# Complexity-ML/complexity-tokenizer

Measured on AMD Instinct MI355X. Metric: MB/s raw UTF-8 encoded (encode_batch), 50k ByteLevel BPE, 1/2/4/8 MI355X, higher is better.
Workload: dtype u8

## Files before the change

### complexity-tokenizer_amd/csrc/ctok_host.cpp

```cpp
#include <emmintrin.h>
#include <sched.h>
#include <hip/hip_runtime.h>

#include <algorithm>
#include <atomic>
#include <chrono>
#include <cstdio>
#include <cstring>
#include <exception>
#include <fstream>
#include <functional>
#include <map>
#include <memory>
#include <mutex>
#include <sstream>
#include <thread>
#include <string>
#include <string_view>
#include <unordered_map>
#include <unordered_set>
#include <vector>

#include "../../include/ctok.h"
#include "ctok_internal.h"
// ... 239 lines not shown
      (void)hipSetDevice(device);
      if (pipe) {
        for (int i = 0; i < 2; i++) {
          if (pipe->ev_h2d[i]) (void)hipEventDestroy(pipe->ev_h2d[i]);
          if (pipe->ev_enc[i]) (void)hipEventDestroy(pipe->ev_enc[i]);
          if (pipe->ev_d2h[i]) (void)hipEventDestroy(pipe->ev_d2h[i]);
        }
        for (auto& e : pipe->ev_t) if (e) (void)hipEventDestroy(e);
        if (pipe->up) (void)hipStreamDestroy(pipe->up);
        if (pipe->down) (void)hipStreamDestroy(pipe->down);
        pipe.reset();
      }
      for (auto& e : ev) if (e) (void)hipEventDestroy(e);
      for (auto& e : dev_ev) if (e) (void)hipEventDestroy(e);
      if (ev_sync) (void)hipEventDestroy(ev_sync);
      if (ev_join) (void)hipEventDestroy(ev_join);
      if (side) (void)hipStreamDestroy(side);
      if (ev_tot) (void)hipEventDestroy(ev_tot);
      if (host) (void)hipHostFree(host);
      if (stream) (void)hipStreamDestroy(stream);
    }
  }
};

}


struct ctok {
  std::unordered_map<std::string, uint32_t> vocab;
  std::unordered_map<uint32_t, std::string> id_to_token;
  std::vector<std::pair<std::string, uint32_t>> special;
  bool nfc = true;
  bool add_prefix_space = false;
  std::vector<uint64_t> merge_tab;
  uint32_t merge_mask = 0;
  std::vector<uint64_t> lds_image;
  std::vector<uint64_t> lds16_image, merge16;
  uint32_t merge16_mask = 0;
  std::vector<uint32_t> pair0;
  size_t hot_entries = 0;
  std::vector<uint32_t> piece_tab;
  uint32_t piece_mask = 0;
  std::vector<uint32_t> rank_newid;
  std::vector<uint32_t> eager_bits;
  std::vector<uint32_t> wmeta;
  bool window = false;
  int32_t byte2id[256];
  std::string at_bytes;
  std::vector<uint32_t> at_off{0}, at_id;
  std::vector<uint8_t> at_flags;
  bool proper = true;
  bool compact = false;
  bool narrow = false;
  bool ids16 = false;
  int decoder = 1;
  std::string decoder_name;
  std::vector<uint32_t> dec_ent;
  std::vector<uint8_t> dec_bytes;
  bool has_pp = false;
  std::vector<uint32_t> pp_items;
  int pp_kind = 0;
  std::string pp_single, pp_pair;
  bool pp_has_pair = false;
  uint64_t model_max_length = 512;
  std::mutex dev_mu;
  std::map<int, std::unique_ptr<DeviceState>> devs;
};

namespace {

bool get_bool_field(const ctj::Value& o, const char* k, bool dflt, const char* ctx) {
  const ctj::Value* v = o.get(k);
  if (!v) return dflt;
  if (v->kind != ctj::Value::Bool) throw_err(CTOK_E_PARSE, std::string("invalid type for `") + k + "` in " + ctx + ", expected a boolean");
  return v->b;
}

int parse_normalizer(const ctj::Value* v) {
  if (v && v->kind == ctj::Value::Object) {
    const ctj::Value* t = v->get("type");
    if (t) {
      std::string ty = t->kind == ctj::Value::String ? t->s : "";
      if (ty == "NFC") return 1;
      if (ty == "Sequence") {
        const ctj::Value* ns = v->get("normalizers");
        if (!ns || ns->kind != ctj::Value::Array) return 0;
        int any = 0;
        for (const auto& n : ns->arr) any |= parse_normalizer(&n);
        return any;
      }
      static const char* unsup[] = {"NFD", "NFKC", "NFKD", "Lowercase", "Strip", "StripAccents", "Replace",
                                    "Prepend", "BertNormalizer", "Precompiled"};
      for (const char* u : unsup)
        if (ty == u) throw_err(CTOK_E_UNSUPPORTED, "normalizer `" + ty + "` is outside the encode hot path (only NFC / none)");
      return 0;
    }
  }
  return 1;
}

bool is_white_space(uint32_t c) {
  return (c >= 9 && c <= 13) || c == 32 || c == 0x85 || c == 0xA0 || c == 0x1680 || (c >= 0x2000 && c <= 0x200A) ||
         c == 0x2028 || c == 0x2029 || c == 0x202F || c == 0x205F || c == 0x3000;
}

std::string encode_utf8(const std::vector<uint32_t>& cps, size_t a, size_t b) {
// ... 653 lines not shown
          const uint32_t v = t->compact ? z : r;
          t->eager_bits[v >> 5] |= 1u << (v & 31);
        }
      }
    }
  }


  {
    auto nchars = [&](uint32_t id, bool& ok) -> uint32_t {
      auto it = t->id_to_token.find(id);
      if (it == t->id_to_token.end()) { ok = false; return 0; }
      uint32_t c = 0;
      for (unsigned char ch : it->second) c += (ch & 0xC0) != 0x80;
      return c;
    };
    bool ok = !getenv("CTOK_NO_WINDOW");
    for (int b = 0; b < 256 && ok; b++)
      if (t->byte2id[b] >= 0 && nchars((uint32_t)t->byte2id[b], ok) != 1) ok = false;
    uint32_t max_id = 0;
    for (const auto& kv : t->vocab) max_id = std::max(max_id, kv.second);
    std::vector<uint32_t> ml, mr;
    if (ok) {
      ml.assign((size_t)max_id + 1, 0);
      mr.assign((size_t)max_id + 1, 0);
    }
    for (const auto& kv : ranks) {
      if (!ok) break;
      const uint32_t r = kv.second;
      if (r >= valid_new.size()) continue;
      const uint32_t a = (uint32_t)(kv.first >> 32), b = (uint32_t)kv.first;
      const uint32_t la = nchars(a, ok), lb = nchars(b, ok), lz = nchars(valid_new[r], ok);
      if (!ok || lz != la + lb || a > max_id || b > max_id) { ok = false; break; }
      ml[b] = std::max(ml[b], la);
      mr[a] = std::max(mr[a], lb);
    }
    t->window = ok;
    if (ok) {
      t->wmeta.resize((size_t)max_id + 1);
      for (size_t i = 0; i <= max_id; i++) t->wmeta[i] = std::min(ml[i], 0xFFFFu) | std::min(mr[i], 0xFFFFu) << 16;
    }
  }
  lap("window");

  t->pair0.assign(65536, kNoRank);
  for (uint32_t a = 0; a < 256; a++)
    for (uint32_t b = 0; b < 256; b++) {
      if (t->byte2id[a] < 0 || t->byte2id[b] < 0) continue;
      auto it = ranks.find(((uint64_t)(uint32_t)t->byte2id[a] << 32) | (uint32_t)t->byte2id[b]);
      if (it == ranks.end()) continue;
      const uint32_t r = it->second;
      t->pair0[a * 256 + b] = t->compact ? (r < valid_new.size() ? valid_new[r] : kPanicVal) : r;
    }

  lap("proper+pair0");
  {
    std::vector<int> inv0(0x144, -1);
    for (int b = 0; b < 256; b++) inv0[bm[b]] = b;
    auto tab_value = [&](uint32_t a, uint32_t b) -> uint64_t {
      const uint64_t key = ((uint64_t)a << kIdBits) | b;
      for (uint32_t h = mhash(a, b) & t->merge_mask;; h = (h + 1) & t->merge_mask) {
        const uint64_t e = t->merge_tab[h];
        if (e == kEmpty) return UINT64_MAX;
        if ((e & ((1ull << 42) - 1)) == key) return e >> 42;
      }
    };
    const uint64_t n_valid = valid_new.size();
    auto panics = [&](uint64_t v) { return t->compact ? v == kPanicVal : v >= n_valid; };
    std::vector<std::pair<const std::string*, uint32_t>> items;
    items.reserve(t->vocab.size());
    for (const auto& kv : t->vocab) items.push_back({&kv.first, kv.second});
    const unsigned nth = std::min(16u, usable_cpus_once());
    std::vector<std::vector<std::pair<std::string, uint32_t>>> part(nth);
    auto work = [&](unsigned w) {
      std::vector<uint32_t> cps, tk;
      for (size_t i = w; i < items.size(); i += nth) {
        const std::string& key = *items[i].first;
        if (!decode_utf8(key, cps) || cps.empty() || cps.size() > 8) continue;
        std::string raw;
        bool ok = true;
        for (uint32_t c : cps) {
          if (c >= inv0.size() || inv0[c] < 0) { ok = false; break; }
          raw += (char)inv0[c];
        }
        if (!ok) continue;
        tk.clear();
        for (unsigned char c : raw) {
          if (t->byte2id[c] < 0) { ok = false; break; }
          tk.push_back((uint32_t)t->byte2id[c]);
        }
        if (!ok) continue;
        for (;;) {
          size_t bi = 0;
          uint64_t best = UINT64_MAX;
          for (size_t j = 0; j + 1 < tk.size(); j++) {
            const uint64_t v = tab_value(tk[j], tk[j + 1]);
            if (v == UINT64_MAX) continue;
            if (panics(v)) { ok = false; break; }
            if (v < best) { best = v; bi = j; }
          }
          if (!ok || best == UINT64_MAX) break;
          tk[bi] = t->compact ? (uint32_t)best : valid_new[best];
          tk.erase(tk.begin() + bi + 1);
        }
        if (ok && tk.size() == 1 && tk[0] == items[i].second) part[w].push_back({raw, items[i].second});
      }
// ... 166 lines not shown
      return b;
    }();
    upload(ds->cls_bmp, bmp.data(), bmp.size(), s);
  }
  upload(ds->decomp_cp, ct_decomp_cp, CT_DECOMP_N, s);
  upload(ds->decomp_off, ct_decomp_off, CT_DECOMP_N + 1, s);
  upload(ds->decomp_data, ct_decomp_data, CT_DECOMP_DATA_N, s);
  upload(ds->comp_key, (const uint64_t*)ct_comp_key, CT_COMP_N, s);
  upload(ds->comp_val, ct_comp_val, CT_COMP_N, s);
  upload(ds->alnum, ct_bytemap_alnum, 256, s);
  upload(ds->at_bytes, (const uint8_t*)t->at_bytes.data(), t->at_bytes.size(), s);
  upload(ds->at_off, t->at_off.data(), t->at_off.size(), s);
  upload(ds->at_id, t->at_id.data(), t->at_id.size(), s);
  upload(ds->at_flags, t->at_flags.data(), t->at_flags.size(), s);
  HIPTRY(hipStreamSynchronize(s));
  Tables& tb = ds->t;
  tb.merge_tab = ds->merge_tab.p;
  tb.merge_mask = t->merge_mask;
  tb.lds_image = (const uint4*)ds->lds_image.p;
  tb.pair0 = ds->pair0.p;
  tb.lds16_image = (const uint4*)ds->lds16_image.p;
  tb.merge16 = ds->merge16.p;
  tb.merge16_mask = t->merge16_mask;
  tb.piece_tab = (const uint4*)ds->piece_tab.p;
  tb.piece_mask = t->piece_mask;
  tb.rank_newid = ds->rank_newid.p;
  tb.eager = ds->eager.p;
  tb.wmeta = ds->wmeta.p;
  tb.window = t->window ? 1 : 0;
  tb.n_ranks = (uint32_t)t->rank_newid.size();
  tb.byte2id = ds->byte2id.p;
  tb.cls_s1 = ds->cls_s1.p;
  tb.cls_s2 = ds->cls_s2.p;
  tb.nfc_s1 = ds->nfc_s1.p;
  tb.nfc_s2 = ds->nfc_s2.p;
  tb.cls_bmp = ds->cls_bmp.p;
  tb.cp_fast = cp_fast_ok() ? 1u : 0u;
  tb.decomp_cp = ds->decomp_cp.p;
  tb.decomp_off = ds->decomp_off.p;
  tb.decomp_data = ds->decomp_data.p;
  tb.n_decomp = CT_DECOMP_N;
  tb.comp_key = ds->comp_key.p;
  tb.comp_val = ds->comp_val.p;
  tb.n_comp = CT_COMP_N;
  tb.bytemap_alnum = ds->alnum.p;
  tb.at_bytes = ds->at_bytes.p;
  tb.at_off = ds->at_off.p;
  tb.at_id = ds->at_id.p;
  tb.at_flags = ds->at_flags.p;
  tb.n_at = (uint32_t)t->at_id.size();
  tb.proper = (t->proper && !getenv("CTOK_FORCE_IMPROPER")) ? 1 : 0;
  tb.compact = t->compact ? 1 : 0;
  tb.narrow = (t->narrow && !getenv("CTOK_FORCE_WIDE_SLOTS")) ? 1 : 0;
  tb.all_bytes = std::all_of(t->byte2id, t->byte2id + 256, [](int32_t v) { return v >= 0; }) ? 1 : 0;
  tb.dbg = getenv("CTOK_DBG_MODE") ? (uint32_t)atoi(getenv("CTOK_DBG_MODE")) : 0;
  DeviceState* r = ds.get();
  t->devs[device] = std::move(ds);
  return r;
}

bool debug_sync() {
  static int v = -1;
  if (v < 0) v = getenv("CTOK_DEBUG_SYNC") ? 1 : 0;
  return v == 1;
}

#define STEP(name, x)                                                                    \
  do {                                                                                   \
    HIPTRY(x);                                                                           \
    if (debug_sync()) {                                                                  \
      fprintf(stderr, "[ctok] %s launched\n", name);                                     \
      HIPTRY(hipStreamSynchronize(s));                                                   \
      fprintf(stderr, "[ctok] %s done\n", name);                                         \
    }                                                                                    \
  } while (0)

template <class Idle>
void spin_sync(DeviceState* ds, hipStream_t s, Idle idle) {
  HIPTRY(hipEventRecord(ds->ev_sync, s));
  for (;;) {
    hipError_t e = hipEventQuery(ds->ev_sync);
    if (e == hipSuccess) return;
    if (e != hipErrorNotReady) throw_err(CTOK_E_DEVICE, std::string("hipEventQuery: ") + hipGetErrorString(e));
    idle();
  }
}
void spin_sync(DeviceState* ds, hipStream_t s) {
  spin_sync(ds, s, [] {});
}

struct Laps {
  struct Lap {
    hipEvent_t a, b;
    double v;
    bool done;
  };
  Lap l[12];
  int n = 0;
  int add(hipEvent_t a, hipEvent_t b) {
    l[n] = {a, b, 0.0, false};
    return n++;
  }
  void read(Lap& p) {
    float v = 0;
    HIPTRY(hipEventElapsedTime(&v, p.a, p.b));
    p.v = v;
// ... 1615 lines not shown
```

### complexity-tokenizer_amd/csrc/ctok_internal.h

```cpp
#pragma once
#include <hip/hip_runtime.h>

#include <cstdint>

namespace ctok_dev {

constexpr uint64_t kEmpty = ~0ull;
constexpr uint32_t kIdBits = 21;
constexpr uint64_t kKeyMask = (1ull << 42) - 1;
constexpr uint32_t kNoRank = 0x3FFFFFu;
constexpr uint32_t kMaxId = (1u << kIdBits) - 2;
constexpr uint32_t kPanicVal = kNoRank - 1;

constexpr uint32_t kErrPanic = 1u;

constexpr int kTileWords = 62;
constexpr int kTile = kTileWords * 64;
constexpr int kTileSlots = 4096;
constexpr int kSegWaves = 4;
constexpr int kSegUnroll = 4;
constexpr int kShortMax = 32;
constexpr int kMedMax = 64;
constexpr uint32_t kCap0 = kTile, kCap1 = (kTile + 8) / 9, kCap2 = (kTile + 16) / 17, kCap3 = (kTile + 32) / 33;
constexpr uint32_t kCap0Lean = 1040;
// ... 73 lines not shown
  uint32_t h = mul24(lo, 0x9E3779u) + mul24((lo >> 24) | (hi << 8), 0x85EBCBu) + mul24((hi >> 16) | (len << 16), 0xC2B2AFu);
  h ^= h >> 15;
  h = mul24(h, 0x27D4EBu) ^ (h >> 9);
  return h ^ (h >> 16);
}

__host__ __device__ __forceinline__ int cp_range_class(uint32_t cp) {
  if (cp - 0x4E00u < 0x5200u) return 1;
  if (cp - 0xAC00u < 0x2BA4u) return 1;
  if (cp - 0x3041u < 0x56u) return 1;
  if (cp - 0x30A1u < 0x5Au) return 1;
  if (cp - 0x1F300u < 0x350u) return 3;
  return -1;
}

struct Tables {
  const uint64_t* merge_tab;
  uint32_t merge_mask;
  const uint4* lds_image;
  const uint32_t* pair0;
  const uint4* lds16_image;
  const uint64_t* merge16;
  uint32_t merge16_mask;
  const uint4* piece_tab;
  uint32_t piece_mask;
  const uint32_t* rank_newid;
  uint32_t n_ranks;
  const int32_t* byte2id;
  const uint8_t* cls_s1;
  const uint8_t* cls_s2;
  const uint8_t* nfc_s1;
  const uint16_t* nfc_s2;
  const uint8_t* cls_bmp;
  uint32_t cp_fast;
  const uint32_t* decomp_cp;
  const uint16_t* decomp_off;
  const uint32_t* decomp_data;
  uint32_t n_decomp;
  const uint64_t* comp_key;
  const uint32_t* comp_val;
  uint32_t n_comp;
  const uint8_t* bytemap_alnum;
  const uint8_t* at_bytes;
  const uint32_t* at_off;
  const uint32_t* at_id;
  const uint8_t* at_flags;
  uint32_t n_at;
  uint32_t proper;
  const uint32_t* eager;
  uint32_t window;
  const uint32_t* wmeta;
  uint32_t compact;
  uint32_t narrow;
  uint32_t dbg;
  uint32_t all_bytes;
};

struct Work {
  const uint8_t* text;
  uint32_t n_bytes;
  const uint64_t* doc_off;
  uint32_t n_docs;
  uint32_t* tfirst;
  uint32_t* pbits;
  uint32_t n_words;
  uint32_t n_tiles;
  uint32_t n_cus;
  uint32_t nfc_watch;
  uint32_t* nfc_bits;
  uint32_t mid_wide;
  uint32_t short_wgs;
  uint32_t keep_first;
  uint16_t* wpref;
  uint32_t* tile_np;
  uint32_t* tile_tok;
  uint32_t* tile_doc;
  uint32_t* tcls;
  uint32_t* list0;
  uint32_t k0;
  uint32_t* list1;
  uint32_t* list2;
  uint32_t* list3;
  void* prec;
  uint32_t rec16;
  uint32_t* mrec;
  uint32_t* pdoc;
  uint32_t* tcnt;
  uint32_t* long_cnt;
  uint32_t* long_ord;
  uint32_t* long_hist;
  uint32_t* scratch;
  uint32_t* lids;
  uint32_t* long_pos;
  uint32_t* lw_pos;
  uint32_t* rend;
  uint2* tregion;
  uint32_t long_cap, mid_cap;
  uint32_t unit;
  uint64_t* long_list;
  uint64_t* mid_list;
  uint32_t* counters;
  uint32_t* lw;
  uint32_t* scan_tmp;
  uint64_t scan_tmp_cap;
  uint64_t* stamps;
  uint32_t c3_max;
// ... 112 lines not shown
```

### complexity-tokenizer_amd/csrc/kernels.hip

```cpp
#include <hip/hip_ext.h>
#include <hip/hip_runtime.h>

#include <algorithm>
#include <mutex>
#include <type_traits>

#include "ctok_internal.h"
#include "seg_lane.h"

namespace ctok_dev {

#define HIPCHK(x) do { hipError_t e_ = (x); if (e_ != hipSuccess) return e_; } while (0)

template <typename F, typename... A>
static void launch_lx(const Lx& x, F k, dim3 grid, dim3 block, uint32_t lds, hipStream_t s, A... a) {
  if (x.start || x.stop)
    hipExtLaunchKernelGGL(k, grid, block, lds, s, x.start, x.stop, 0u, a...);
  else
    hipLaunchKernelGGL(k, grid, block, lds, s, a...);
}

constexpr uint32_t kNone = 0xFFFFFFFFu;
constexpr uint32_t kDead = 0xFFFFFFFFu;
constexpr uint32_t kSel = kNoRank - 1;


__device__ __forceinline__ void write_report(const Work& w) {
  const uint32_t lane = threadIdx.x & 63;
  uint32_t c3 = 0;
  if (w.c3_max) {
    const uint32_t c = w.counters[kNumCounters + lane];
    uint32_t inc = c;
#pragma unroll
    for (int o = 1; o < 64; o <<= 1) {
      const uint32_t v = (uint32_t)__shfl_up((int)inc, o, 64);
      if (lane >= (uint32_t)o) inc += v;
    }
    w.c3pre[lane] = inc - c;
    if (lane == 63) w.c3pre[64] = inc;
    c3 = __shfl((int)inc, 63, 64);
    if (__ballot(c > w.c3_max / kC3Shards)) c3 = ~0u;
  }
  if (lane < (uint32_t)kNumCounters) w.report[lane] = lane == (uint32_t)kCtrC3Count ? c3 : w.counters[lane];
  __builtin_amdgcn_fence(__ATOMIC_RELEASE, "");
  asm volatile("s_waitcnt vmcnt(0)" ::: "memory");
  if (lane == 0) __hip_atomic_store(&w.report[kNumCounters], w.seq, __ATOMIC_RELAXED, __HIP_MEMORY_SCOPE_SYSTEM);
  __builtin_amdgcn_fence(__ATOMIC_RELEASE, "");
}

__device__ __forceinline__ uint32_t wave_min_u32(uint32_t v) {
#pragma unroll
  for (int o = 32; o > 0; o >>= 1) v = min(v, (uint32_t)__shfl_xor((int)v, o, 64));
  return v;
}

__device__ __forceinline__ uint32_t wave_min_full_u32(uint32_t v) {
  v = min(v, (uint32_t)__builtin_amdgcn_update_dpp((int)v, (int)v, 0xB1, 0xF, 0xF, false));
  v = min(v, (uint32_t)__builtin_amdgcn_update_dpp((int)v, (int)v, 0x4E, 0xF, 0xF, false));
  v = min(v, (uint32_t)__builtin_amdgcn_update_dpp((int)v, (int)v, 0x141, 0xF, 0xF, false));
  v = min(v, (uint32_t)__builtin_amdgcn_update_dpp((int)v, (int)v, 0x140, 0xF, 0xF, false));
// ... 1052 lines not shown
template <> struct LdsClass<32> { static constexpr int cls = 2; static constexpr uint32_t cap = kCap2; };
template <> struct LdsClass<64> { static constexpr int cls = 3; static constexpr uint32_t cap = kCap3; };

template <int N>
__device__ __forceinline__ const uint32_t* class_list(const Work& w) {
  return N == 8 ? w.list0 : N == 16 ? w.list1 : N == 32 ? w.list2 : w.list3;
}
template <int N>
__device__ __forceinline__ uint32_t class_cap(const Work& w) {
  return N == 8 ? w.k0 : LdsClass<N>::cap;
}

template <int N, bool COMPACT, bool HOT, bool NARROW>
__device__ __forceinline__ bool merge_slots(const Tables& t, const PairLds& P, uint32_t* tk, uint32_t* rk,
                                            uint32_t& m, uint32_t stop, uint32_t* err) {
  for (;;) {
    if (m <= stop) return true;
    uint32_t key = ~0u;
#pragma unroll
    for (int k = 0; k < N - 1; k++) key = min(key, (rk[k] << 6) | (uint32_t)k);
    const uint32_t best = key >> 6, bi = key & 63u;
    if (best == kNoRank) return false;
    const uint32_t nid = COMPACT ? best : t.rank_newid[best];
    uint32_t L = 0, R = 0;
#pragma unroll
    for (int k = 0; k < N; k++) {
      L = ((uint32_t)k + 1 == bi) ? tk[k] : L;
      R = ((uint32_t)k == bi + 2) ? tk[k] : R;
    }
    const bool has_l = bi > 0, has_r = bi + 2 < m;
    Probe<NARROW, HOT> pl, pr;
    pl.start(t, P, L, nid, has_l);
    pr.start(t, P, nid, R, has_r);
#pragma unroll
    for (int k = 0; k < N; k++) {
      const uint32_t nxt_t = k + 1 < N ? tk[k + 1] : kDead;
      const uint32_t nxt_r = k + 1 < N ? rk[k + 1] : kNoRank;
      const bool gt = (uint32_t)k > bi;
      tk[k] = gt ? nxt_t : ((uint32_t)k == bi ? nid : tk[k]);
      rk[k] = gt ? nxt_r : rk[k];
    }
    m--;
    const uint32_t rl = has_l ? pl.finish(t, err) : kNoRank;
    const uint32_t rr = has_r ? pr.finish(t, err) : kNoRank;
#pragma unroll
    for (int k = 0; k < N - 1; k++)
      rk[k] = ((uint32_t)k + 1 == bi) ? rl : (((uint32_t)k == bi) ? rr : rk[k]);
  }
}

typedef __attribute__((address_space(3))) uint16_t lds_u16;

template <bool COMPACT, bool HOT, uint32_t NT, typename OutOf>
__device__ __forceinline__ uint32_t merge_lds8(const Tables& t, const PairLds& P, const uint32_t* tk, const uint32_t* rk,
                                               uint32_t m, lds_u32* s_key, lds_u16* s_tok, uint32_t* err,
                                               OutOf&& out_of) {
  const uint32_t tid = threadIdx.x;
#pragma unroll
  for (int k = 0; k < 8; k++) {
    s_key[k * NT + tid] = (uint32_t)k + 1 < m ? (rk[k] << 3) | (uint32_t)k : ~0u;
    s_tok[k * NT + tid] = (uint16_t)tk[k];
  }
  uint32_t lv = ((1u << m) - 1u) | 0x100u;
  for (;;) {
    uint32_t kk[8];
#pragma unroll
    for (int k = 0; k < 8; k++) kk[k] = s_key[k * NT + tid];
    const uint32_t best = min(min(min(kk[0], kk[1]), min(kk[2], kk[3])), min(min(kk[4], kk[5]), min(kk[6], kk[7])));
    if (best >= (kNoRank << 3)) break;
    const uint32_t bi = best & 7u, r = best >> 3;
    const uint32_t nid = (COMPACT ? r : t.rank_newid[r]) & 0xFFFFu;
    const uint32_t p = bi + 1 + (uint32_t)__builtin_ctz(lv >> (bi + 1));
    const uint32_t q = p + 1 + (uint32_t)__builtin_ctz(lv >> (p + 1));
    const bool has_r = q < 8;
    const uint32_t lo = lv & ((1u << bi) - 1u);
    const bool has_l = lo != 0;
    const uint32_t pv = 31u - (uint32_t)__builtin_clz(lo | 1u);
    const uint32_t L = s_tok[pv * NT + tid], R = s_tok[min(q, 7u) * NT + tid];
    s_tok[bi * NT + tid] = (uint16_t)nid;
    s_key[p * NT + tid] = ~0u;
    lv &= ~(1u << p);
    m--;
    Probe<true, HOT> pl, pr;
    pl.start(t, P, L, nid, has_l);
    pr.start(t, P, nid, R, has_r);
    const uint32_t rl = pl.finish(t, err), rr = pr.finish(t, err);
    if (has_l) s_key[pv * NT + tid] = (rl << 3) | pv;
    s_key[bi * NT + tid] = has_r ? (rr << 3) | bi : ~0u;
  }
  uint32_t* out = out_of(m);
#pragma unroll
  for (int k = 0; k < 8; k++)
    if ((lv >> k) & 1u) out[__popc(lv & ((1u << k) - 1u))] = s_tok[k * NT + tid];
  return m;
}

template <uint32_t SORTCAP, int KT = 64>
struct PassLds {
  uint32_t pre[KT + 1], tsum[KT], tbase[KT], stat[2], bcnt[4], bfill[4], chunk, take, next;
  uint16_t perm[SORTCAP];
};

template <int N, bool COMPACT, bool HOT, uint32_t NT, uint32_t SORTCAP, bool L8 = false, int KT = 64, typename Load>
__device__ __forceinline__ void class_pass(const Work& w, const Tables& t, const PairLds& P, const int32_t* s_b2id,
                                           PassLds<SORTCAP, KT>& S, bool& loaded, Load&& load,
                                           lds_u32* s_key = nullptr, lds_u16* s_tok = nullptr) {
  using LC = LdsClass<N>;
  constexpr int K = KT;
  static_assert(KT <= (int)NT, "a thread per chunk tile");
  const uint32_t tid = threadIdx.x;
  uint32_t* err = &w.counters[2];
  const uint32_t* list = class_list<N>(w);
  const uint32_t cap = class_cap<N>(w);
  const uint32_t* counts = w.tcls + (size_t)LC::cls * w.n_tiles;
  uint32_t st_bytes = 0, st_ids = 0;
  if (tid < 2) S.stat[tid] = 0;
  constexpr uint32_t blo = N == 8 ? 1 : N / 2 + 1, bw = N == 64 ? 8 : N == 32 ? 4 : 2;
  auto bucket = [&](uint32_t n) { return min(3u, (n - blo) / bw); };
  __syncthreads();
  uint32_t take = 1;
  const uint32_t U = w.unit;
  for (;;) {
    if (tid == 0) {
      S.chunk = atomicAdd(&w.counters[ctr_chunk(LC::cls)], take);
      S.take = take;
      S.next = 0;
    }
    __syncthreads();
    const uint32_t c0 = S.chunk * U;
    if (c0 >= w.n_tiles) break;
    const uint32_t tb1 = min(w.n_tiles, c0 + U * S.take);
    const uint32_t E = tile_share_init<K>(counts, tb1, c0, S.pre, S.tsum, w.tregion, LC::cls, S.tbase);
    if (E && !loaded) {
      load();
      loaded = true;
      __syncthreads();
    }
    const bool sorted = N > 8 && E <= SORTCAP;
    if (sorted) {
      if (tid < 4) { S.bcnt[tid] = 0; S.bfill[tid] = 0; }
      __syncthreads();
      for (uint32_t q = tid; q < E; q += NT) {
        const uint32_t kt = tile_of<K>(S.pre, q);
        const uint32_t b = bucket(ent_len(list[(size_t)(c0 + kt) * cap + (q - S.pre[kt])]));
#pragma unroll
        for (uint32_t bb = 0; bb < 4; bb++) {
          const uint64_t m = __ballot(b == bb);
          if (m && (threadIdx.x & 63) == __ffsll((unsigned long long)m) - 1) atomicAdd(&S.bcnt[bb], (uint32_t)__popcll(m));
        }
      }
      __syncthreads();
      if (tid == 0) {
        uint32_t acc = 0;
        for (int bb = 0; bb < 4; bb++) {
          const uint32_t c = S.bcnt[bb];
          S.bfill[bb] = acc;
          acc += c;
        }
      }
      __syncthreads();
      for (uint32_t q = tid; q < E; q += NT) {
        const uint32_t kt = tile_of<K>(S.pre, q);
        const uint32_t b = bucket(ent_len(list[(size_t)(c0 + kt) * cap + (q - S.pre[kt])]));
#pragma unroll
        for (uint32_t bb = 0; bb < 4; bb++) {
          const uint32_t slot = wave_append(&S.bfill[bb], b == bb);
          if (b == bb) S.perm[slot] = (uint16_t)q;
        }
      }
      __syncthreads();
    }
    auto entry = [&](uint32_t i, uint32_t& kt) {
      const uint32_t q = sorted ? (uint32_t)S.perm[i] : i;
      kt = tile_of<K>(S.pre, q);
      return list[(size_t)(c0 + kt) * cap + (q - S.pre[kt])];
    };
    auto start_of = [&](uint32_t e, uint32_t kt) { return (c0 + kt) * kTile + (e & 0xFFFu); };
    auto body = [&](uint32_t e, uint32_t kt, const uint32_t* wv, auto&& hook) {
        const uint32_t tile = c0 + kt;
        const uint32_t s = tile * kTile + (e & 0xFFFu);
        const uint32_t o = ent_ord(e);
        const uint32_t n = ent_len(e);
        uint32_t tk[N], rk[N];
        bool missing = false;
        {
#pragma unroll
          for (int k = 0; k < N; k++) {
            const int32_t id = s_b2id[byte_of(wv[k >> 2], k)];
            missing |= ((uint32_t)k < n) & (id < 0);
            tk[k] = (uint32_t)id;
          }
        }
        if (missing) {
          hook();
          const uint32_t mi = atomicAdd(&w.counters[4], 1u);
          if (mi < w.mid_cap)
            w.mid_list[mi] = (uint64_t)s | ((uint64_t)o << 32) | ((uint64_t)n << 48);
          else
            atomicOr(&w.counters[kCtrOverflow], 1u);
          return;
        }
        {
          uint32_t bytes[N];
#pragma unroll
          for (int k = 0; k < N; k++) bytes[k] = byte_of(wv[k >> 2], k);
#pragma unroll
          for (int k = 0; k < N - 1; k++) rk[k] = t.pair0[(bytes[k] << 8) | bytes[k + 1]];
#pragma unroll
          for (int k = 0; k < N - 1; k++) {
            const bool live = (uint32_t)k + 1 < n;
            if (live && rk[k] != kNoRank && value_panics(t, rk[k])) atomicOr(err, kErrPanic);
            rk[k] = (live && !(rk[k] != kNoRank && value_panics(t, rk[k]))) ? rk[k] : kNoRank;
          }
        }
        rk[N - 1] = kNoRank;
        uint32_t m = n;
        bool more = true;
        if constexpr (N >= 64) more = merge_slots<64, COMPACT, HOT, L8>(t, P, tk, rk, m, 32, err);
        if constexpr (N >= 32) {
          if (more) more = merge_slots<32, COMPACT, HOT, L8>(t, P, tk, rk, m, 16, err);
        }
        if constexpr (N >= 16) {
          if (more) more = merge_slots<16, COMPACT, HOT, L8>(t, P, tk, rk, m, 8, err);
        }
        hook();
        uint32_t pos = 0;
        auto out_of = [&](uint32_t mm) {
          pos = atomicAdd(&S.tsum[kt], mm);
          return w.scratch + (size_t)tile * kTileSlots + pos;
        };
        if (L8 && more) {
          m = merge_lds8<COMPACT, HOT, NT>(t, P, tk, rk, m, s_key, s_tok, err, out_of);
        } else {
          if (!L8 && more) merge_slots<8, COMPACT, HOT, L8>(t, P, tk, rk, m, 0, err);
          uint32_t* out = out_of(m);
// ... 54 lines not shown
      while (b0 < E) {
        const uint32_t i = b0 + lane;
        const uint32_t b2 = b1 < E ? take() : E;
        const uint32_t e = e0, kt = kt0;
        uint32_t wv[kPw];
#pragma unroll
        for (int k = 0; k < kPw; k++) wv[k] = __builtin_amdgcn_alignbyte(d0[k + 1], d0[k], sh0);
        e0 = e1;
        kt0 = kt1;
        if (b1 + lane < E) issue_words(start_of(e0, kt0));
        if (b2 + lane < E) e1 = entry(b2 + lane, kt1);
        b0 = b1;
        b1 = b2;
        if (i < E) body(e, kt, wv, hook);
        else hook();
      }
    }
    tile_share_flush<K>(w, c0, tb1, S.tsum, S.tbase, LC::cls);
    const uint32_t units = (w.n_tiles + U - 1) / U, next = S.chunk + S.take;
    const uint32_t share = next < units ? (units - next) / gridDim.x : 0u;
    take = min(min((uint32_t)K / U, max(1u, share)), N <= 16 ? 64u : max(1u, (2 * NT * S.take + E) / (E + 1)));
    __syncthreads();
  }
#pragma unroll
  for (int o = 32; o > 0; o >>= 1) {
    st_bytes += (uint32_t)__shfl_xor((int)st_bytes, o, 64);
    st_ids += (uint32_t)__shfl_xor((int)st_ids, o, 64);
  }
  if ((tid & 63) == 0) {
    atomicAdd(&S.stat[0], st_bytes);
    atomicAdd(&S.stat[1], st_ids);
  }
  __syncthreads();
  if (tid == 0) {
    atomicAdd(&w.counters[ctr_stat(LC::cls)], S.stat[0]);
    atomicAdd(&w.counters[ctr_stat(LC::cls) + 1], S.stat[1]);
  }
  __syncthreads();
}


#ifndef CTOK_SHORT_NT
#define CTOK_SHORT_NT 1024
#endif
#ifndef CTOK_SHORT_SORTCAP
#define CTOK_SHORT_SORTCAP 7168
#endif
template <bool NARROW> struct ShortCfg {
  static constexpr uint32_t NT = NARROW ? CTOK_SHORT_NT : 1024;
  static constexpr uint32_t SORTCAP = NARROW ? CTOK_SHORT_SORTCAP : kSortCap;
};
constexpr int kShortKT = 64;

template <bool COMPACT, bool NARROW>
__global__ __launch_bounds__(1024) void k_bpe_short(Work w, Tables t, uint32_t passes) {
  if (w.report && blockIdx.x == 0 && threadIdx.x < 64) write_report(w);
  if (spec_failed(w)) return;
  constexpr uint32_t NT = ShortCfg<NARROW>::NT;
  extern __shared__ __attribute__((aligned(16))) uint4 s_img[];
  __shared__ int32_t s_b2id[256];
  __shared__ PassLds<ShortCfg<NARROW>::SORTCAP, kShortKT> S;
  __shared__ uint32_t s_key[NARROW ? 8 * NT : 1];
  __shared__ uint16_t s_tok[NARROW ? 8 * NT : 1];
  const uint32_t tid = threadIdx.x;
  const uint4* img = NARROW ? t.lds16_image : t.lds_image;
  auto load = [&] {
    for (uint32_t i = tid; i < kLdsImageBytes / 16; i += NT) s_img[i] = img[i];
    for (uint32_t i = tid; i < 256; i += NT) s_b2id[i] = t.byte2id[i];
  };
  bool loaded = false;
  const PairLds P{(const lds_u64*)s_img, (const lds_u32*)(s_img + kHotBuckets)};
  lds_u32* sk = (lds_u32*)s_key;
  lds_u16* st = (lds_u16*)s_tok;
  WgRec::begin(w.wgrec, 0);
  if (passes & 1u)
    class_pass<8, COMPACT, true, NT, ShortCfg<NARROW>::SORTCAP, NARROW, kShortKT>(w, t, P, s_b2id, S, loaded, load, sk, st);
  if (passes & 2u)
    class_pass<16, COMPACT, true, NT, ShortCfg<NARROW>::SORTCAP, NARROW, kShortKT>(w, t, P, s_b2id, S, loaded, load, sk, st);
  WgRec::end(w.wgrec, 0, loaded ? 1u : 0u);
}


template <bool COMPACT, bool NARROW>
__device__ __forceinline__ uint32_t merge_wave64(const Tables& t, const PairLds& P, uint32_t& tok, uint32_t rk,
                                                 uint64_t& lv, uint32_t* err) {
  const uint32_t lane = threadIdx.x & 63;
  for (;;) {
    const uint32_t best = wave_min_full_u32((rk << 6) | lane);
    const uint32_t r = best >> 6, bi = best & 63u;
    if (r == kNoRank) break;
    const uint32_t nid = COMPACT ? r : uni(t.rank_newid[r]);
    const uint64_t right = lv & ~((2ull << bi) - 1ull);
    const uint32_t p = (uint32_t)__builtin_ctzll(right);
    const uint64_t after = right & (right - 1ull);
    const bool has_r = after != 0;
    const uint32_t q = has_r ? (uint32_t)__builtin_ctzll(after) : 0u;
    const uint64_t left = lv & ((1ull << bi) - 1ull);
    const bool has_l = left != 0;
    const uint32_t pv = has_l ? 63u - (uint32_t)__builtin_clzll(left) : 0u;
    const uint32_t L = __builtin_amdgcn_readlane(tok, pv), R = __builtin_amdgcn_readlane(tok, q);
    uint32_t v = kNoRank;
    if (lane < 2) {
      Probe<NARROW, true> pr;
      pr.start(t, P, lane == 0 ? L : nid, lane == 0 ? nid : R, lane == 0 ? has_l : has_r);
      v = pr.finish(t, err);
    }
    const uint32_t rl = __builtin_amdgcn_readlane(v, 0), rr = __builtin_amdgcn_readlane(v, 1);
    tok = lane == bi ? nid : tok;
    rk = (has_l && lane == pv) ? rl : rk;
    rk = lane == bi ? (has_r ? rr : kNoRank) : rk;
    rk = lane == p ? kNoRank : rk;
    lv &= ~(1ull << p);
  }
  return (uint32_t)__popcll(lv);
}

template <bool COMPACT, bool NARROW>
__device__ __forceinline__ void sparse_c3(const Work& w, const Tables& t, const PairLds& P, const int32_t* s_b2id,
                                          uint32_t n) {
  const uint32_t lane = threadIdx.x & 63;
  const uint32_t cap = w.c3_max / kC3Shards;
  const uint32_t pre = w.c3pre[lane];
  uint32_t* err = &w.counters[2];
  uint32_t st_bytes = 0, st_ids = 0;
  for (;;) {
    const uint32_t k = uni(atomicAdd(&w.counters[kCtrC3Take], lane == 0 ? 1u : 0u));
    if (k >= n) break;
    const uint32_t sh = 63u - (uint32_t)__builtin_clzll(__ballot(pre <= k));
    const uint32_t qe = uni(w.c3q[(size_t)sh * cap + (k - __builtin_amdgcn_readlane(pre, sh))]);
    const uint32_t tile = qe >> 7;
    const uint32_t e = uni(w.list3[(size_t)tile * kCap3 + (qe & 127u)]);
// ... 78 lines not shown
  __syncthreads();
  if (!s_left) {
    if constexpr (CLS == 2) WgRec::end(w.wgrec, 1, 0);
    return;
  }
  const uint32_t tid = threadIdx.x;
  const uint4* img = NARROW ? t.lds16_image : t.lds_image;
  for (uint32_t i = tid; i < kLdsImageBytes / 16; i += NT) s_img[i] = img[i];
  for (uint32_t i = tid; i < 256; i += NT) s_b2id[i] = t.byte2id[i];
  bool loaded = true;
  const PairLds P{(const lds_u64*)s_img, (const lds_u32*)(s_img + kHotBuckets)};
  class_pass<CLS == 2 ? 32 : 64, COMPACT, true, NT, kSortCap, NARROW, KT>(w, t, P, s_b2id, S, loaded, [] {},
                                                                         (lds_u32*)s_key, (lds_u16*)s_tok);
  if constexpr (CLS == 2) WgRec::end(w.wgrec, 1, 1);
}

struct LdsAttr {
  std::mutex mu;
  uint64_t done = 0;
};
static hipError_t lds_attr_once(LdsAttr& a, const void* fn, size_t bytes) {
  int dev = 0;
  HIPCHK(hipGetDevice(&dev));
  const uint64_t bit = dev < 64 ? 1ull << dev : 0ull;
  std::lock_guard<std::mutex> lk(a.mu);
  if (a.done & bit) return hipSuccess;
  HIPCHK(hipFuncSetAttribute(fn, hipFuncAttributeMaxDynamicSharedMemorySize, (int)bytes));
  a.done |= bit;
  return hipSuccess;
}

template <bool C, int CLS, bool NW>
static hipError_t launch_mid_t(const Work& w, const Tables& t, hipStream_t s, const Lx& x) {
  static LdsAttr attr;
  HIPCHK(lds_attr_once(attr, (const void*)k_bpe_mid<C, CLS, NW>, kLdsImageBytes));
  if (!w.n_tiles) return hipSuccess;
  const uint32_t grid = min((w.n_tiles + w.unit - 1) / w.unit, w.n_cus);
  if constexpr (CLS == 2) {
    if (w.mid_wide) {
      static LdsAttr attr768;
      HIPCHK(lds_attr_once(attr768, (const void*)k_bpe_mid<C, CLS, NW, 768>, kLdsImageBytes));
      launch_lx(x, k_bpe_mid<C, CLS, NW, 768>, grid, 768, kLdsImageBytes, s, w, t);
      return hipGetLastError();
    }
  }
  launch_lx(x, k_bpe_mid<C, CLS, NW>, grid, 512, kLdsImageBytes, s, w, t);
  return hipGetLastError();
}
template <bool C, int CLS>
static hipError_t launch_mid(const Work& w, const Tables& t, hipStream_t s, const Lx& x = {}) {
  return t.narrow ? launch_mid_t<C, CLS, true>(w, t, s, x) : launch_mid_t<C, CLS, false>(w, t, s, x);
}

template <bool C, bool NW>
static hipError_t launch_short_t(const Work& w, const Tables& t, hipStream_t s, const Lx& x) {
  static LdsAttr attr;
  HIPCHK(lds_attr_once(attr, (const void*)k_bpe_short<C, NW>, kLdsImageBytes));
  if (!w.n_tiles) return hipSuccess;
  const uint32_t grid = min((w.n_tiles + w.unit - 1) / w.unit, w.short_wgs ? min(w.short_wgs, w.n_cus) : w.n_cus);
  if (t.dbg == 30) {
    k_bpe_short<C, NW><<<grid, ShortCfg<NW>::NT, kLdsImageBytes, s>>>(w, t, 1u);
    k_bpe_short<C, NW><<<grid, ShortCfg<NW>::NT, kLdsImageBytes, s>>>(w, t, 2u);
  } else {
    launch_lx(x, k_bpe_short<C, NW>, grid, ShortCfg<NW>::NT, kLdsImageBytes, s, w, t, 3u);
  }
  return hipGetLastError();
}
template <bool C>
static hipError_t launch_short(const Work& w, const Tables& t, hipStream_t s, const Lx& x) {
  return t.narrow ? launch_short_t<C, true>(w, t, s, x) : launch_short_t<C, false>(w, t, s, x);
}

template <bool C, bool NW>
static hipError_t launch_sparse_t(const Work& w, const Tables& t, uint32_t n_pieces, hipStream_t s, const Lx& x) {
  static LdsAttr attr;
  HIPCHK(lds_attr_once(attr, (const void*)k_bpe_sparse<C, NW>, kLdsImageBytes));
  const uint32_t grid = std::max(1u, std::min((n_pieces + kSparseWaves - 1) / kSparseWaves, w.n_cus));
  launch_lx(x, k_bpe_sparse<C, NW>, grid, 64 * kSparseWaves, kLdsImageBytes, s, w, t, n_pieces);
  return hipGetLastError();
}

hipError_t launch_c3_sparse(const Work& w, const Tables& t, uint32_t n_pieces, hipStream_t s, Lx x) {
  if (!n_pieces || n_pieces > w.c3_max || !w.n_tiles) return hipSuccess;
  if (t.compact)
    return t.narrow ? launch_sparse_t<true, true>(w, t, n_pieces, s, x) : launch_sparse_t<true, false>(w, t, n_pieces, s, x);
  return t.narrow ? launch_sparse_t<false, true>(w, t, n_pieces, s, x) : launch_sparse_t<false, false>(w, t, n_pieces, s, x);
}

hipError_t launch_bpe_class(const Work& w, const Tables& t, int cls, hipStream_t s, Lx x) {
  if (t.n_at != 0) {
    if (cls == 0 && w.n_tiles)
      launch_lx(x, k_bpe_generic<false>, (w.n_tiles + kTilesGeneric - 1) / kTilesGeneric, 256, 0, s, w, t);
    return hipGetLastError();
  }
  switch (cls) {
    case 0: return t.compact ? launch_short<true>(w, t, s, x) : launch_short<false>(w, t, s, x);
    case 2: return t.compact ? launch_mid<true, 2>(w, t, s, x) : launch_mid<false, 2>(w, t, s, x);
    case 4: return t.compact ? launch_mid<true, 3>(w, t, s, x) : launch_mid<false, 3>(w, t, s, x);
    case 3:
      if (t.all_bytes) return hipSuccess;
      launch_lx(x, k_bpe_generic<true>, 64, 128, 0, s, w, t);
      return hipGetLastError();
    default:
      return hipSuccess;
  }
}


template <bool GMEM>
struct LongState;

template <>
struct LongState<true> {
  uint32_t* tok;
  uint32_t* nxt;
  uint32_t* prv;
  uint32_t* rk;
  static __device__ __forceinline__ uint32_t ld(const uint32_t* p) {
    return __hip_atomic_load(p, __ATOMIC_RELAXED, __HIP_MEMORY_SCOPE_AGENT);
  }
  static __device__ __forceinline__ void st(uint32_t* p, uint32_t v) {
    __hip_atomic_store(p, v, __ATOMIC_RELAXED, __HIP_MEMORY_SCOPE_AGENT);
// ... 1904 lines not shown
```

Measured before the change: 165,900.

## Add packed 16-bit register merge tier for 9..16 byte short pieces

Adds a packed path to the 9..16 byte short-piece class pass. Token ids and ranks are held as pairs of 16-bit halves in eight registers, and the merge loop runs in those registers until the piece shrinks to 8 tokens, then hands off to the existing LDS-based merge. The path is enabled when the narrow and compact tables show every rank fits in 16 bits. It aims to cut LDS traffic and per-merge work for medium-short pieces, at the cost of extra register pressure, shift and select instructions, and another kernel instantiation.

```diff
diff --git a/complexity-tokenizer_amd/csrc/ctok_host.cpp b/complexity-tokenizer_amd/csrc/ctok_host.cpp
--- a/complexity-tokenizer_amd/csrc/ctok_host.cpp
+++ b/complexity-tokenizer_amd/csrc/ctok_host.cpp
@@ -315,6 +315,7 @@
   bool proper = true;
   bool compact = false;
   bool narrow = false;
+  bool short_packed = false;
   bool ids16 = false;
   int decoder = 1;
   std::string decoder_name;
@@ -1074,6 +1075,18 @@
       const uint32_t r = it->second;
       t->pair0[a * 256 + b] = t->compact ? (r < valid_new.size() ? valid_new[r] : kPanicVal) : r;
     }
+  if (t->narrow && t->compact) {
+    auto fits = [&](uint32_t v) { return v < 0xFFFFu; };
+    bool ok = true;
+    for (uint32_t v : t->pair0) ok = ok && (v == kNoRank || fits(v));
+    for (uint64_t e : t->merge16) ok = ok && (e == kEmpty || fits((uint32_t)(e >> 32)));
+    for (uint32_t i = 0; i < kHotU64; i++) {
+      const uint64_t e = t->lds16_image[i];
+      ok = ok && (e == kEmpty || fits((uint32_t)(e >> 32)));
+    }
+    t->short_packed = ok;
+  }
+  if (lt) fprintf(stderr, "[ctok load] narrow %d compact %d short_packed %d\n", (int)t->narrow, (int)t->compact, (int)t->short_packed);
 
   lap("proper+pair0");
   {
@@ -1346,6 +1359,10 @@
   tb.proper = (t->proper && !getenv("CTOK_FORCE_IMPROPER")) ? 1 : 0;
   tb.compact = t->compact ? 1 : 0;
   tb.narrow = (t->narrow && !getenv("CTOK_FORCE_WIDE_SLOTS")) ? 1 : 0;
+  {
+    const char* pk = getenv("CTOK_SHORT_PACKED");
+    tb.short_packed = (tb.narrow && t->short_packed && !(pk && atoi(pk) == 0)) ? 1 : 0;
+  }
   tb.all_bytes = std::all_of(t->byte2id, t->byte2id + 256, [](int32_t v) { return v >= 0; }) ? 1 : 0;
   tb.dbg = getenv("CTOK_DBG_MODE") ? (uint32_t)atoi(getenv("CTOK_DBG_MODE")) : 0;
   DeviceState* r = ds.get();
diff --git a/complexity-tokenizer_amd/csrc/ctok_internal.h b/complexity-tokenizer_amd/csrc/ctok_internal.h
--- a/complexity-tokenizer_amd/csrc/ctok_internal.h
+++ b/complexity-tokenizer_amd/csrc/ctok_internal.h
@@ -149,6 +149,7 @@
   const uint32_t* wmeta;
   uint32_t compact;
   uint32_t narrow;
+  uint32_t short_packed;
   uint32_t dbg;
   uint32_t all_bytes;
 };
diff --git a/complexity-tokenizer_amd/csrc/kernels.hip b/complexity-tokenizer_amd/csrc/kernels.hip
--- a/complexity-tokenizer_amd/csrc/kernels.hip
+++ b/complexity-tokenizer_amd/csrc/kernels.hip
@@ -6,6 +6,7 @@
 #include <type_traits>
 
 #include "ctok_internal.h"
+#include "merge16_hd.h"
 #include "seg_lane.h"
 
 namespace ctok_dev {
@@ -1164,15 +1165,9 @@
 typedef __attribute__((address_space(3))) uint16_t lds_u16;
 
 template <bool COMPACT, bool HOT, uint32_t NT, typename OutOf>
-__device__ __forceinline__ uint32_t merge_lds8(const Tables& t, const PairLds& P, const uint32_t* tk, const uint32_t* rk,
-                                               uint32_t m, lds_u32* s_key, lds_u16* s_tok, uint32_t* err,
-                                               OutOf&& out_of) {
+__device__ __forceinline__ uint32_t merge_lds8_run(const Tables& t, const PairLds& P, uint32_t m, lds_u32* s_key,
+                                                   lds_u16* s_tok, uint32_t* err, OutOf&& out_of) {
   const uint32_t tid = threadIdx.x;
-#pragma unroll
-  for (int k = 0; k < 8; k++) {
-    s_key[k * NT + tid] = (uint32_t)k + 1 < m ? (rk[k] << 3) | (uint32_t)k : ~0u;
-    s_tok[k * NT + tid] = (uint16_t)tk[k];
-  }
   uint32_t lv = ((1u << m) - 1u) | 0x100u;
   for (;;) {
     uint32_t kk[8];
@@ -1207,13 +1202,64 @@
   return m;
 }
 
+template <bool COMPACT, bool HOT, uint32_t NT, typename OutOf>
+__device__ __forceinline__ uint32_t merge_lds8(const Tables& t, const PairLds& P, const uint32_t* tk, const uint32_t* rk,
+                                               uint32_t m, lds_u32* s_key, lds_u16* s_tok, uint32_t* err,
+                                               OutOf&& out_of) {
+  const uint32_t tid = threadIdx.x;
+#pragma unroll
+  for (int k = 0; k < 8; k++) {
+    s_key[k * NT + tid] = (uint32_t)k + 1 < m ? (rk[k] << 3) | (uint32_t)k : ~0u;
+    s_tok[k * NT + tid] = (uint16_t)tk[k];
+  }
+  return merge_lds8_run<COMPACT, HOT, NT>(t, P, m, s_key, s_tok, err, out_of);
+}
+
+template <bool HOT>
+struct Lookup16 {
+  const Tables& t;
+  const PairLds& P;
+  uint32_t* err;
+  Probe<true, HOT> pl, pr;
+  bool has_l = false, has_r = false;
+  __device__ __forceinline__ uint32_t new_id(uint32_t v) const { return v; }
+  __device__ __forceinline__ void start(uint32_t L, uint32_t nid, uint32_t R, bool hl, bool hr) {
+    has_l = hl;
+    has_r = hr;
+    pl.start(t, P, L, nid, hl);
+    pr.start(t, P, nid, R, hr);
+  }
+  __device__ __forceinline__ void finish(uint32_t& rl, uint32_t& rr) {
+    rl = (has_l ? pl.finish(t, err) : kNoRank) & 0xFFFFu;
+    rr = (has_r ? pr.finish(t, err) : kNoRank) & 0xFFFFu;
+  }
+};
+
+template <int K0, int K1, uint32_t NT>
+__device__ __forceinline__ void lds8_store_packed(const uint32_t (&T)[8], const uint32_t (&R)[8], lds_u32* s_key,
+                                                  lds_u16* s_tok) {
+  if constexpr (K0 < K1) {
+    s_key[K0 * NT + threadIdx.x] = m16::lds8_key<K0>(R);
+    s_tok[K0 * NT + threadIdx.x] = (uint16_t)m16::half<K0>(T);
+    lds8_store_packed<K0 + 1, K1, NT>(T, R, s_key, s_tok);
+  }
+}
+template <int K0, int K1>
+__device__ __forceinline__ void store_packed_ids(const uint32_t (&T)[8], uint32_t m, uint32_t* out) {
+  if constexpr (K0 < K1) {
+    if ((uint32_t)K0 < m) out[K0] = m16::half<K0>(T);
+    store_packed_ids<K0 + 1, K1>(T, m, out);
+  }
+}
+
 template <uint32_t SORTCAP, int KT = 64>
 struct PassLds {
   uint32_t pre[KT + 1], tsum[KT], tbase[KT], stat[2], bcnt[4], bfill[4], chunk, take, next;
   uint16_t perm[SORTCAP];
 };
 
-template <int N, bool COMPACT, bool HOT, uint32_t NT, uint32_t SORTCAP, bool L8 = false, int KT = 64, typename Load>
+template <int N, bool COMPACT, bool HOT, uint32_t NT, uint32_t SORTCAP, bool L8 = false, int KT = 64, bool PK = false,
+          typename Load>
 __device__ __forceinline__ void class_pass(const Work& w, const Tables& t, const PairLds& P, const int32_t* s_b2id,
                                            PassLds<SORTCAP, KT>& S, bool& loaded, Load&& load,
                                            lds_u32* s_key = nullptr, lds_u16* s_tok = nullptr) {
@@ -1293,6 +1339,59 @@
         const uint32_t s = tile * kTile + (e & 0xFFFu);
         const uint32_t o = ent_ord(e);
         const uint32_t n = ent_len(e);
+        if constexpr (PK) {
+          static_assert(N == 16 && L8 && COMPACT, "the packed tier is the 9..16 B pass's, ahead of merge_lds8, on compact tables");
+          uint32_t T[8], R[8], bytes[N];
+          bool missing = false;
+#pragma unroll
+          for (int k = 0; k < N; k++) bytes[k] = byte_of(wv[k >> 2], k);
+#pragma unroll
+          for (int d = 0; d < 8; d++) {
+            const int32_t i0 = s_b2id[bytes[2 * d]], i1 = s_b2id[bytes[2 * d + 1]];
+            missing |= (((uint32_t)(2 * d) < n) & (i0 < 0)) | (((uint32_t)(2 * d + 1) < n) & (i1 < 0));
+            T[d] = m16::pack2((uint32_t)i0, (uint32_t)i1);
+          }
+          if (missing) {
+            hook();
+            const uint32_t mi = atomicAdd(&w.counters[4], 1u);
+            if (mi < w.mid_cap)
+              w.mid_list[mi] = (uint64_t)s | ((uint64_t)o << 32) | ((uint64_t)n << 48);
+            else
+              atomicOr(&w.counters[kCtrOverflow], 1u);
+            return;
+          }
+          {
+            uint32_t v[N];
+#pragma unroll
+            for (int k = 0; k < N - 1; k++) v[k] = t.pair0[(bytes[k] << 8) | bytes[k + 1]];
+            v[N - 1] = kNoRank;
+#pragma unroll
+            for (int k = 0; k < N - 1; k++) v[k] = (uint32_t)k + 1 < n ? v[k] : kNoRank;
+#pragma unroll
+            for (int d = 0; d < 8; d++) R[d] = m16::pack2(v[2 * d], v[2 * d + 1]);
+          }
+          uint32_t m = n;
+          Lookup16<HOT> lk{t, P, err};
+          const bool more = m16::tier(T, R, m, 8u, lk);
+          hook();
+          uint32_t pos = 0;
+          auto out_of = [&](uint32_t mm) {
+            pos = atomicAdd(&S.tsum[kt], mm);
+            return w.scratch + (size_t)tile * kTileSlots + pos;
+          };
+          if (more) {
+            lds8_store_packed<0, 8, NT>(T, R, s_key, s_tok);
+            m = merge_lds8_run<COMPACT, HOT, NT>(t, P, m, s_key, s_tok, err, out_of);
+          } else {
+            store_packed_ids<0, N>(T, m, out_of(m));
+          }
+          CTOK_CHECK_REC(m >= 1 && m <= n && pos + m <= (uint32_t)kTileSlots && o < (uint32_t)kTileSlots,
+                         "[ctok check] packed class pass tile %u: record m=%u n=%u pos=%u ordinal=%u\n", tile, m, n, pos, o);
+          w.mrec[(size_t)tile * kTileSlots + o] = rec_short(m, pos);
+          st_bytes += n;
+          st_ids += m;
+          return;
+        }
         uint32_t tk[N], rk[N];
         bool missing = false;
         {
@@ -1453,8 +1552,9 @@
 };
 constexpr int kShortKT = 64;
 
-template <bool COMPACT, bool NARROW>
+template <bool COMPACT, bool NARROW, bool PK16 = false>
 __global__ __launch_bounds__(1024) void k_bpe_short(Work w, Tables t, uint32_t passes) {
+  static_assert((NARROW && COMPACT) || !PK16, "the packed tier needs the narrow tables and compact values");
   if (w.report && blockIdx.x == 0 && threadIdx.x < 64) write_report(w);
   if (spec_failed(w)) return;
   constexpr uint32_t NT = ShortCfg<NARROW>::NT;
@@ -1477,7 +1577,7 @@
   if (passes & 1u)
     class_pass<8, COMPACT, true, NT, ShortCfg<NARROW>::SORTCAP, NARROW, kShortKT>(w, t, P, s_b2id, S, loaded, load, sk, st);
   if (passes & 2u)
-    class_pass<16, COMPACT, true, NT, ShortCfg<NARROW>::SORTCAP, NARROW, kShortKT>(w, t, P, s_b2id, S, loaded, load, sk, st);
+    class_pass<16, COMPACT, true, NT, ShortCfg<NARROW>::SORTCAP, NARROW, kShortKT, PK16>(w, t, P, s_b2id, S, loaded, load, sk, st);
   WgRec::end(w.wgrec, 0, loaded ? 1u : 0u);
 }
 
@@ -1662,22 +1762,25 @@
   return t.narrow ? launch_mid_t<C, CLS, true>(w, t, s, x) : launch_mid_t<C, CLS, false>(w, t, s, x);
 }
 
-template <bool C, bool NW>
+template <bool C, bool NW, bool PK = false>
 static hipError_t launch_short_t(const Work& w, const Tables& t, hipStream_t s, const Lx& x) {
   static LdsAttr attr;
-  HIPCHK(lds_attr_once(attr, (const void*)k_bpe_short<C, NW>, kLdsImageBytes));
+  HIPCHK(lds_attr_once(attr, (const void*)k_bpe_short<C, NW, PK>, kLdsImageBytes));
   if (!w.n_tiles) return hipSuccess;
   const uint32_t grid = min((w.n_tiles + w.unit - 1) / w.unit, w.short_wgs ? min(w.short_wgs, w.n_cus) : w.n_cus);
   if (t.dbg == 30) {
-    k_bpe_short<C, NW><<<grid, ShortCfg<NW>::NT, kLdsImageBytes, s>>>(w, t, 1u);
-    k_bpe_short<C, NW><<<grid, ShortCfg<NW>::NT, kLdsImageBytes, s>>>(w, t, 2u);
+    k_bpe_short<C, NW, PK><<<grid, ShortCfg<NW>::NT, kLdsImageBytes, s>>>(w, t, 1u);
+    k_bpe_short<C, NW, PK><<<grid, ShortCfg<NW>::NT, kLdsImageBytes, s>>>(w, t, 2u);
   } else {
-    launch_lx(x, k_bpe_short<C, NW>, grid, ShortCfg<NW>::NT, kLdsImageBytes, s, w, t, 3u);
+    launch_lx(x, k_bpe_short<C, NW, PK>, grid, ShortCfg<NW>::NT, kLdsImageBytes, s, w, t, 3u);
   }
   return hipGetLastError();
 }
 template <bool C>
 static hipError_t launch_short(const Work& w, const Tables& t, hipStream_t s, const Lx& x) {
+  if constexpr (C) {
+    if (t.narrow && t.short_packed) return launch_short_t<true, true, true>(w, t, s, x);
+  }
   return t.narrow ? launch_short_t<C, true>(w, t, s, x) : launch_short_t<C, false>(w, t, s, x);
 }
 
diff --git a/complexity-tokenizer_amd/csrc/merge16_hd.h b/complexity-tokenizer_amd/csrc/merge16_hd.h
--- /dev/null
+++ b/complexity-tokenizer_amd/csrc/merge16_hd.h
@@ -0,0 +1,100 @@
+#pragma once
+#include <cstdint>
+
+#if defined(__HIPCC__)
+#define M16_HD __host__ __device__ __forceinline__
+#define M16_UNROLL _Pragma("unroll")
+#else
+#define M16_HD inline
+#define M16_UNROLL
+#endif
+
+namespace m16 {
+
+constexpr uint32_t kNone = 0xFFFFu;
+
+M16_HD uint32_t shr16(uint32_t hi, uint32_t lo) {
+#if defined(__HIP_DEVICE_COMPILE__)
+  return __builtin_amdgcn_alignbyte(hi, lo, 2u);
+#else
+  return (lo >> 16) | (hi << 16);
+#endif
+}
+M16_HD uint32_t umin(uint32_t a, uint32_t b) { return a < b ? a : b; }
+M16_HD uint32_t pack2(uint32_t lo, uint32_t hi) { return (lo & 0xFFFFu) | (hi << 16); }
+M16_HD uint32_t bfi(uint32_t mask, uint32_t a, uint32_t b) { return (a & mask) | (b & ~mask); }
+
+template <int K>
+M16_HD uint32_t half(const uint32_t (&A)[8]) {
+  return (K & 1) ? A[K >> 1] >> 16 : A[K >> 1] & 0xFFFFu;
+}
+M16_HD uint32_t min_key(const uint32_t (&R)[8]) {
+  uint32_t key = ~0u;
+M16_UNROLL
+  for (int d = 0; d < 8; d++) {
+    key = umin(key, (R[d] << 16) | (uint32_t)(2 * d));
+    key = umin(key, (R[d] & 0xFFFF0000u) | (uint32_t)(2 * d + 1));
+  }
+  return key;
+}
+
+template <class LK>
+M16_HD bool step(uint32_t (&T)[8], uint32_t (&R)[8], uint32_t& m, LK& lk) {
+  const uint32_t key = min_key(R);
+  const uint32_t best = key >> 16, bi = key & 15u;
+  if (best == kNone) return false;
+  const uint32_t nid = lk.new_id(best) & 0xFFFFu;
+  const uint32_t D = bi >> 1;
+  const bool odd = (bi & 1u) != 0;
+  uint32_t S[8];
+M16_UNROLL
+  for (int d = 0; d < 8; d++) S[d] = shr16(d + 1 < 8 ? T[d + 1] : ~0u, T[d]);
+  uint32_t A[9];
+  A[0] = odd ? T[0] : 0u;
+M16_UNROLL
+  for (int d = 1; d < 8; d++) A[d] = odd ? T[d] : S[d - 1];
+  A[8] = odd ? ~0u : S[7];
+  uint32_t L0 = 0, R0 = 0;
+M16_UNROLL
+  for (int d = 0; d < 8; d++) {
+    L0 = D == (uint32_t)d ? A[d] : L0;
+    R0 = D == (uint32_t)d ? A[d + 1] : R0;
+  }
+  const uint32_t L = L0 & 0xFFFFu, Rt = R0 >> 16;
+  const bool has_l = bi > 0, has_r = bi + 2 < m;
+  lk.start(L, nid, Rt, has_l, has_r);
+  const uint32_t Y = odd ? (L | (nid << 16)) : (nid | (R0 & 0xFFFF0000u));
+  const uint32_t mA = odd ? 0xFFFFFFFFu : 0x0000FFFFu, mB = odd ? 0u : 0xFFFF0000u;
+  uint32_t mask[8];
+M16_UNROLL
+  for (int d = 0; d < 8; d++) {
+    const bool right = bi < (uint32_t)(2 * d + 1);
+    T[d] = D == (uint32_t)d ? Y : (right ? S[d] : T[d]);
+    const uint32_t sr = shr16(d + 1 < 8 ? R[d + 1] : ~0u, R[d]);
+    R[d] = right ? sr : R[d];
+    mask[d] = D == (uint32_t)d ? mA : (D == (uint32_t)(d + 1) ? mB : 0u);
+  }
+  m--;
+  uint32_t rl, rr;
+  lk.finish(rl, rr);
+  const uint32_t vv = odd ? pack2(rl, rr) : pack2(rr, rl);
+M16_UNROLL
+  for (int d = 0; d < 8; d++) R[d] = bfi(mask[d], vv, R[d]);
+  return true;
+}
+
+template <class LK>
+M16_HD bool tier(uint32_t (&T)[8], uint32_t (&R)[8], uint32_t& m, uint32_t stop, LK& lk) {
+  for (;;) {
+    if (m <= stop) return true;
+    if (!step(T, R, m, lk)) return false;
+  }
+}
+
+template <int K>
+M16_HD uint32_t lds8_key(const uint32_t (&R)[8]) {
+  const uint32_t r = half<K>(R);
+  return r == kNone ? ~0u : (r << 3) | (uint32_t)K;
+}
+
+}
```

Result: faster. 168,800 (median of 6 runs) (+1.8%).
